# iammcy/BFLC-demo

Measured on AMD Instinct MI355X. Metric: fl_round_wall_clock_ms, lower is better.
Workload: dtype bf16; 1 GPU; model=femnist_cnn, global_batch=4096, img=1x28x28x62cls, parallelism=fl_nodes1, clients=8, update_quota=4, aggregate_top_k=3, samples_per_client=3072, batch_size=1024, partition=dirichlet, byzantine_clients=0

## Files before the change

### csrc/hip/bindings.cpp

```cpp
#include <torch/extension.h>

#include <string>
#include <tuple>
#include <vector>

namespace bflc {

void axpy_(torch::Tensor y, torch::Tensor x, double alpha);
void sgd_step_(torch::Tensor p, torch::Tensor g, double lr);
void adam_step_(torch::Tensor p, torch::Tensor g, torch::Tensor m,
                torch::Tensor v, long step, double lr, double beta1,
                double beta2, double eps);
torch::Tensor weighted_fedavg(torch::Tensor deltas, torch::Tensor w);
void sgd_master_(torch::Tensor p, torch::Tensor shadow, torch::Tensor g,
                 double lr);
void adam_master_(torch::Tensor p, torch::Tensor shadow, torch::Tensor g,
                  torch::Tensor m, torch::Tensor v, long step, double lr,
                  double beta1, double beta2, double eps);
void adam_master_graph_(torch::Tensor p, torch::Tensor shadow,
                        torch::Tensor g, torch::Tensor m, torch::Tensor v,
                        torch::Tensor step, torch::Tensor bc, double lr,
                        double beta1, double beta2, double eps);
void refresh_shadow_(torch::Tensor p, torch::Tensor shadow);
void score_load_(torch::Tensor shadow, torch::Tensor global_flat,
// ... 54 lines not shown
std::string conv_fwd_pool_impl(std::vector<long> x_shape,
                               std::vector<long> w_shape, long stride,
                               long pad);
long halo_conv_group_images_query(std::vector<long> x_shape,
                                  std::vector<long> w_shape, long stride,
                                  long pad);
std::string conv2d_relu_pool_route(std::vector<long> x_shape,
                                   std::vector<long> w_shape, long stride,
                                   long pad);
PlanRow conv_plan_route(const std::string& entry, std::vector<long> x_shape,
                        std::vector<long> w_shape, long stride, long pad);
std::tuple<torch::Tensor, torch::Tensor> conv2d_relu_pool_fwd_idx(
    torch::Tensor x, torch::Tensor w, torch::Tensor b, long stride,
    long pad, long max_blocks, std::string impl);
std::tuple<torch::Tensor, torch::Tensor> pool_relu_bwd_colsum(
    torch::Tensor y_pooled, torch::Tensor idx, torch::Tensor dy_pooled,
    std::vector<long> out_shape);
std::tuple<torch::Tensor, torch::Tensor> thin_conv_pool_wgrad(
    torch::Tensor x, torch::Tensor y_pooled, torch::Tensor idx,
    torch::Tensor dy_pooled, long stride, long pad);
std::tuple<torch::Tensor, torch::Tensor> thin_conv_pool_wgrad_fused(
    torch::Tensor x, torch::Tensor y_pooled, torch::Tensor idx,
    torch::Tensor dy_pooled, long stride, long pad);
std::string thin_pool_wgrad_impl(std::vector<long> x_shape,
                                 std::vector<long> w_shape, long stride,
                                 long pad, bool want_dx);
std::string conv2d_relu_pool_bwd_route(std::vector<long> x_shape,
                                       std::vector<long> w_shape,
                                       long stride, long pad, bool want_dx,
                                       bool allow_direct);
std::tuple<torch::Tensor, torch::Tensor, torch::Tensor> conv2d_relu_pool_bwd(
    torch::Tensor x, torch::Tensor w, torch::Tensor y_pooled,
    torch::Tensor idx, torch::Tensor dy_pooled, long stride, long pad,
    bool want_db, bool want_dx, bool allow_direct);

std::tuple<torch::Tensor, torch::Tensor, torch::Tensor> batchnorm_fwd(
    torch::Tensor x, torch::Tensor gamma, torch::Tensor beta, double eps,
    bool relu, c10::optional<torch::Tensor> residual);
std::tuple<torch::Tensor, torch::Tensor, torch::Tensor> batchnorm_bwd(
    torch::Tensor x, torch::Tensor dy, torch::Tensor mean,
    torch::Tensor invstd, torch::Tensor gamma,
    c10::optional<torch::Tensor> y_relu);
torch::Tensor global_avgpool_fwd(torch::Tensor x);
torch::Tensor global_avgpool_bwd(torch::Tensor dy, long H, long W);
torch::Tensor add_relu_fwd(torch::Tensor a, torch::Tensor b);
torch::Tensor add_relu_bwd(torch::Tensor y, torch::Tensor dy);

std::tuple<torch::Tensor, torch::Tensor, torch::Tensor> groupnorm_fwd(
    torch::Tensor x, torch::Tensor gamma, torch::Tensor beta, long groups,
    double eps, bool relu, c10::optional<torch::Tensor> residual);
std::tuple<torch::Tensor, torch::Tensor, torch::Tensor> groupnorm_bwd(
    torch::Tensor x, torch::Tensor dy, torch::Tensor mean, torch::Tensor rstd,
    torch::Tensor gamma, long groups, c10::optional<torch::Tensor> y_relu);
std::string groupnorm_route(long H, long W, long C, long groups);

}

PYBIND11_MODULE(TORCH_EXTENSION_NAME, m) {
  m.doc() = "bflc_amd hand-written gfx950 (CDNA4) HIP kernels";
  m.def("axpy_", &bflc::axpy_, "y += alpha*x (fp32, in place)");
  m.def("sgd_step_", &bflc::sgd_step_, "fused flat SGD");
  m.def("adam_step_", &bflc::adam_step_, "fused flat Adam");
  m.def("weighted_fedavg", &bflc::weighted_fedavg,
        "fixed-order weighted FedAvg reduce");
  m.def("sgd_master_", &bflc::sgd_master_,
        "fused fp32-master SGD + bf16 shadow refresh");
  m.def("adam_master_", &bflc::adam_master_);
// ... 83 lines not shown
        "route conv2d_relu_pool_fwd takes: gemm256_pool | thin_pool | "
        "unfused",
        py::arg("x_shape"), py::arg("w_shape"), py::arg("stride"),
        py::arg("pad"));
  m.def("conv2d_relu_pool_fwd_idx", &bflc::conv2d_relu_pool_fwd_idx,
        "training conv + bias + ReLU + 2x2/2 maxpool: (y_pooled, idx), "
        "same routes and options as conv2d_relu_pool_fwd",
        py::arg("x"), py::arg("w"), py::arg("b"), py::arg("stride"),
        py::arg("pad"), py::arg("max_blocks") = 0, py::arg("impl") = "");
  m.def("pool_relu_bwd_colsum", &bflc::pool_relu_bwd_colsum,
        "unpool + ReLU mask + bias grad in one pass: (dy_full_masked, db)",
        py::arg("y_pooled"), py::arg("idx"), py::arg("dy_pooled"),
        py::arg("out_shape"));
  m.def("thin_conv_pool_wgrad", &bflc::thin_conv_pool_wgrad,
        "direct first-layer (dw, db) from the pooled tensors",
        py::arg("x"), py::arg("y_pooled"), py::arg("idx"),
        py::arg("dy_pooled"), py::arg("stride"), py::arg("pad"));
  m.def("thin_conv_pool_wgrad_fused", &bflc::thin_conv_pool_wgrad_fused,
        "first-layer (dw, db) from the pooled tensors, bitwise the "
        "materialised unpool -> im2col -> split-K GEMM chain",
        py::arg("x"), py::arg("y_pooled"), py::arg("idx"),
        py::arg("dy_pooled"), py::arg("stride"), py::arg("pad"));
  m.def("thin_pool_wgrad_impl", &bflc::thin_pool_wgrad_impl,
        "what the unpool route runs for the thin first layer: "
        "fused_mfma | materialized",
        py::arg("x_shape"), py::arg("w_shape"), py::arg("stride"),
        py::arg("pad"), py::arg("want_dx"));
  m.def("conv2d_relu_pool_bwd_route", &bflc::conv2d_relu_pool_bwd_route,
        "route conv2d_relu_pool_bwd takes: thin_direct | unpool",
        py::arg("x_shape"), py::arg("w_shape"), py::arg("stride"),
        py::arg("pad"), py::arg("want_dx"), py::arg("allow_direct") = true);
  m.def("conv2d_relu_pool_bwd", &bflc::conv2d_relu_pool_bwd,
        "(dx, dw, db) of the fused conv + ReLU + pool from its saved "
        "(x, w, y_pooled, idx)",
        py::arg("x"), py::arg("w"), py::arg("y_pooled"), py::arg("idx"),
        py::arg("dy_pooled"), py::arg("stride"), py::arg("pad"),
        py::arg("want_db") = true, py::arg("want_dx") = true,
        py::arg("allow_direct") = true);
  m.def("batchnorm_fwd", &bflc::batchnorm_fwd,
        py::arg("x"), py::arg("gamma"), py::arg("beta"), py::arg("eps"),
        py::arg("relu"), py::arg("residual") = py::none(),
        "(y, mean, invstd) — batch-stats BN, optional fused relu");
  m.def("batchnorm_bwd", &bflc::batchnorm_bwd, "(dx, dgamma, dbeta)",
        py::arg("x"), py::arg("dy"), py::arg("mean"), py::arg("invstd"),
        py::arg("gamma"), py::arg("y_relu") = py::none());
  m.def("global_avgpool_fwd", &bflc::global_avgpool_fwd);
  m.def("global_avgpool_bwd", &bflc::global_avgpool_bwd);
  m.def("add_relu_fwd", &bflc::add_relu_fwd, "fused residual add + relu");
  m.def("add_relu_bwd", &bflc::add_relu_bwd);
  m.def("groupnorm_fwd", &bflc::groupnorm_fwd,
        py::arg("x"), py::arg("gamma"), py::arg("beta"), py::arg("groups"),
        py::arg("eps"), py::arg("relu"), py::arg("residual") = py::none(),
        "(y, mean [N,G], rstd [N,G]) — per-sample GroupNorm, optional "
        "fused residual add + relu");
  m.def("groupnorm_bwd", &bflc::groupnorm_bwd, "(dx, dgamma, dbeta)",
        py::arg("x"), py::arg("dy"), py::arg("mean"), py::arg("rstd"),
        py::arg("gamma"), py::arg("groups"), py::arg("y_relu") = py::none());
  m.def("groupnorm_route", &bflc::groupnorm_route,
        "route groupnorm_fwd/bwd take: slab | split (from H, W, C, groups "
        "only — never N)",
        py::arg("H"), py::arg("W"), py::arg("C"), py::arg("groups"));
}
```

### csrc/hip/conv2d.hip

```cpp

#include "common.h"
#include "gemm_api.h"

namespace bflc {

namespace {

typedef __attribute__((ext_vector_type(8))) __bf16 bf16x8_t;
typedef __attribute__((ext_vector_type(8))) unsigned short u16x8_t;
typedef __attribute__((ext_vector_type(8))) int i32x8_t;
typedef __attribute__((ext_vector_type(4))) float f32x4_t;

__global__ void im2col_nhwc_vec_kernel(const bf16* __restrict__ x,
                                       bf16* __restrict__ col, ConvShape sh,
                                       long total_g) {
  const int c8g = sh.C / 8;
  const int rs = sh.R * sh.S;
  long g = (long)blockIdx.x * blockDim.x + threadIdx.x;
  const long stride = (long)gridDim.x * blockDim.x;
  for (; g < total_g; g += stride) {
    const int c8 = (int)(g % c8g) * 8;
    const int k = (int)((g / c8g) % rs);
    const long m = g / ((long)c8g * rs);
    const int s = k % sh.S, r = k / sh.S;
// ... 787 lines not shown

torch::Tensor conv2d_fwd(torch::Tensor x, torch::Tensor w, torch::Tensor b,
                         long stride, long pad, bool relu) {
  return std::get<0>(conv2d_fwd_col(x, w, b, stride, pad, relu, false));
}

std::tuple<torch::Tensor, torch::Tensor, torch::Tensor, torch::Tensor>
conv2d_fwd_bn(torch::Tensor x, torch::Tensor w, long stride, long pad) {
  CHECK_GPU(x); CHECK_CONTIG(x); CHECK_CONTIG(w);
  auto sh = make_shape(x, w, stride, pad);
  auto w2 = w.view({(long)sh.Kout, sh.RSC()});
  auto y = torch::empty({(long)sh.N, (long)sh.OH, (long)sh.OW,
                         (long)sh.Kout}, x.options());
  std::pair<torch::Tensor, torch::Tensor> stats;
  auto none = torch::empty({0}, x.options());
  if (is_1x1_s1(sh)) {
    auto col = x.view({sh.M(), (long)sh.C});
    gemm_bf16_raw(col, w2, y, sh.M(), sh.Kout, sh.RSC(), false, true,
                  nullptr, false, EpStore::kPlain, 0, &stats);
    return {y, col, stats.first.defined() ? stats.first : none,
            stats.second.defined() ? stats.second : none};
  }
  if (gemm_conv_fwd_raw(x, w2, y, sh, nullptr, false, &stats))
    return {y, none, stats.first.defined() ? stats.first : none,
            stats.second.defined() ? stats.second : none};
  auto col = im2col(x, sh);
  const long kp = col.size(1);
  gemm_bf16_raw(col, pad_w2(w2, kp), y, sh.M(), sh.Kout, kp, false, true,
                nullptr, false, EpStore::kPlain, 0, &stats);
  return {y, col, stats.first.defined() ? stats.first : none,
          stats.second.defined() ? stats.second : none};
}

std::tuple<torch::Tensor, torch::Tensor, torch::Tensor> conv2d_bwd(
    torch::Tensor x, torch::Tensor w, torch::Tensor dy, long stride,
    long pad, c10::optional<torch::Tensor> col_cache, bool want_db,
    bool want_dx) {
  CHECK_GPU(x); CHECK_CONTIG(x); CHECK_CONTIG(w); CHECK_CONTIG(dy);
  auto sh = make_shape(x, w, stride, pad);
  auto w2 = w.view({(long)sh.Kout, sh.RSC()});
  auto dy2 = dy.view({sh.M(), (long)sh.Kout});

  torch::Tensor dx;
  bool dgrad_done = !want_dx;
  if (!want_dx) {
    dx = torch::empty({0}, x.options());
  } else if (is_1x1_s1(sh)) {
    auto wT = transpose_bf16(w2);
    dx = torch::empty_like(x);
    auto dxv = dx.view({sh.M(), (long)sh.C});
    gemm_bf16_raw(dy2, wT, dxv, sh.M(), sh.RSC(), sh.Kout, false, true,
                  nullptr, false, EpStore::kPlain, 0);
    dgrad_done = true;
  } else if (sh.Kout % 8 == 0 && sh.C <= dgrad_implicit_max_c() &&
             sh.C >= 8 && sh.stride == 1) {
    auto wrot2 = w.permute({3, 1, 2, 0}).contiguous()
                     .view({(long)sh.C, (long)sh.R * sh.S * sh.Kout});
    dx = torch::empty_like(x);
    auto dxv = dx.view({(long)sh.N * sh.H * sh.W, (long)sh.C});
    dgrad_done = gemm_conv_dgrad_raw(dy2, wrot2, dxv, sh);
  }
  if (!dgrad_done) {
    auto wT = transpose_bf16(w2);
    auto dcol = torch::empty({sh.M(), sh.RSC()}, x.options());
    gemm_bf16_raw(dy2, wT, dcol, sh.M(), sh.RSC(), sh.Kout, false, true,
                  nullptr, false, EpStore::kPlain, 0);
    dx = torch::empty_like(x);
    if (sh.C % 8 == 0) {
      const long total_g = (long)sh.N * sh.H * sh.W * (sh.C / 8);
      hipLaunchKernelGGL(col2im_nhwc_vec_kernel, dim3(ew_grid(total_g)),
                         dim3(256), 0, cur_stream(),
                         (const bf16*)dcol.data_ptr(),
                         (bf16*)dx.data_ptr(), sh, total_g);
    } else {
      const long total = dx.numel();
      hipLaunchKernelGGL(col2im_nhwc_kernel, dim3(ew_grid(total)), dim3(256),
                         0, cur_stream(), (const bf16*)dcol.data_ptr(),
                         (bf16*)dx.data_ptr(), sh, total);
    }
    HIP_CHECK(hipGetLastError());
  }

  auto dw = torch::empty_like(w2);
  bool wgrad_done = false;
  if (!is_1x1_s1(sh) && sh.Kout <= wgrad_implicit_max_kout() &&
      !(col_cache.has_value() && col_cache->numel() > 0))
    wgrad_done = gemm_conv_wgrad_raw(dy2, x, dw, sh);
  if (!wgrad_done) {
    auto col = (col_cache.has_value() && col_cache->numel() > 0)
                   ? *col_cache
                   : (is_1x1_s1(sh) ? x.view({sh.M(), (long)sh.C})
                                    : im2col(x, sh));
    const long kp = col.size(1);
    if (kp == sh.RSC()) {
      gemm_bf16_raw(dy2, col, dw, sh.Kout, sh.RSC(), sh.M(), true, false,
                    nullptr, false, EpStore::kPlain, 0);
    } else {
      auto dwp = torch::empty({(long)sh.Kout, kp}, dw.options());
      gemm_bf16_raw(dy2, col, dwp, sh.Kout, kp, sh.M(), true, false,
                    nullptr, false, EpStore::kPlain, 0);
      dw.copy_(dwp.slice(1, 0, sh.RSC()));
    }
  }

  auto db = want_db ? colsum_bf16(dy2)
                    : torch::empty({0}, dy.options());
  return {dx, dw.view(w.sizes()), db};
}

std::tuple<torch::Tensor, torch::Tensor> maxpool2d_fwd(torch::Tensor x,
                                                       long kernel,
                                                       long stride,
                                                       bool want_idx) {
  CHECK_GPU(x); CHECK_CONTIG(x);
  ConvShape sh;
  sh.N = (int)x.size(0); sh.H = (int)x.size(1);
  sh.W = (int)x.size(2); sh.C = (int)x.size(3);
  sh.R = sh.S = (int)kernel; sh.stride = (int)stride; sh.pad = 0;
  sh.Kout = sh.C;
  sh.OH = (sh.H - sh.R) / sh.stride + 1;
  sh.OW = (sh.W - sh.S) / sh.stride + 1;
  auto y = torch::empty({(long)sh.N, (long)sh.OH, (long)sh.OW, (long)sh.C},
                        x.options());
  TORCH_CHECK(sh.R * sh.S <= 255, "maxpool window too large for u8 idx");
  const bool skip_idx = !want_idx && sh.C % 8 == 0;
  auto idx = skip_idx
                 ? torch::empty({0}, y.options().dtype(at::kByte))
                 : torch::empty_like(y, y.options().dtype(at::kByte));
  if (sh.C % 8 == 0) {
    const long total_g = sh.M() * (sh.C / 8);
    hipLaunchKernelGGL(maxpool_nhwc_vec_fwd, dim3(ew_grid(total_g)),
                       dim3(256), 0, cur_stream(),
                       (const bf16*)x.data_ptr(), (bf16*)y.data_ptr(),
                       skip_idx ? nullptr : idx.data_ptr<uint8_t>(), sh,
                       total_g);
  } else {
    const long total = y.numel();
    hipLaunchKernelGGL(maxpool_nhwc_fwd, dim3(ew_grid(total)), dim3(256), 0,
                       cur_stream(), (const bf16*)x.data_ptr(),
                       (bf16*)y.data_ptr(), idx.data_ptr<uint8_t>(), sh,
// ... 121 lines not shown
  bool ok = false;
  long S = 1, kslice = 0;
  int tbl_pairs = 0;
  long lds = 0;
  int cshift = 0;
};

ThinFusedPlan thin_fused_plan(const ConvShape& sh) {
  ThinFusedPlan t;
  if (!thin_wgrad_eligible(sh) || sh.N <= 0) return t;
  const long Mpix = sh.M();
  const long kp = (sh.RSC() + 7) / 8 * 8;
  const GemmPlan p = gemm_dense_plan(sh.Kout, kp, Mpix, true, false);
  const long lim = 1L << 31;
  if (p.path != GemmPath::kSmall || kp != 16 || Mpix * sh.Kout >= lim ||
      (long)sh.N * sh.H * sh.W >= lim || (long)sh.N * (sh.OH + 2) >= lim)
    return t;
  t.S = p.S;
  t.kslice = p.kslice;
  int rows_max = 0;
  for (long s = 0; s < p.S; ++s) {
    int P0, rows;
    thin_wgrad_window(sh, s * p.kslice,
                      std::min(Mpix, (s + 1) * p.kslice), &P0, &rows);
    rows_max = std::max(rows_max, rows);
  }
  const long xelems = (long)(rows_max + 2) * (sh.OW + 2) + 4;
  const long pairs = (p.kslice / 32 + 1) * 16;
  t.tbl_pairs = (int)pairs;
  t.lds = pairs * 8 + (xelems + 1) / 2 * 4;
  while (t.cshift < 6 && (1 << t.cshift) < sh.OW + 2) ++t.cshift;
  t.ok = t.lds <= kThinFusedMaxLds && xelems <= 32768;
  return t;
}

}

torch::Tensor conv2d_relu_pool_fwd(torch::Tensor x, torch::Tensor w,
                                   torch::Tensor b, long stride, long pad,
                                   long max_blocks, std::string impl) {
  return std::get<0>(
      relu_pool_fwd_impl(x, w, b, stride, pad, false, max_blocks, impl));
}

std::string conv_fwd_pool_impl(std::vector<long> x_shape,
                               std::vector<long> w_shape, long stride,
                               long pad) {
  const auto sh = make_shape_dims(x_shape, w_shape, stride, pad);
  return pool_route(sh) == PoolRoute::kGemm256 && halo_conv_gate(sh)
             ? "halo_mfma"
             : "gemm256";
}

long halo_conv_group_images_query(std::vector<long> x_shape,
                                  std::vector<long> w_shape, long stride,
                                  long pad) {
  return halo_conv_group_images(
      make_shape_dims(x_shape, w_shape, stride, pad));
}

std::tuple<torch::Tensor, torch::Tensor> conv2d_relu_pool_fwd_idx(
    torch::Tensor x, torch::Tensor w, torch::Tensor b, long stride,
    long pad, long max_blocks, std::string impl) {
  return relu_pool_fwd_impl(x, w, b, stride, pad, true, max_blocks, impl);
}

// ... 57 lines not shown
                     (const bf16*)y_pooled.data_ptr(),
                     idx.data_ptr<uint8_t>(),
                     (const bf16*)dy_pooled.data_ptr(), sh, MP, G, rows,
                     part.data_ptr<float>());
  HIP_CHECK(hipGetLastError());
  hipLaunchKernelGGL(thin_conv_pool_wgrad_final_kernel,
                     dim3(ceil_div((long)N * kWgradAcc, 4)), dim3(256), 0,
                     cur_stream(), part.data_ptr<float>(), chunks, N,
                     (bf16*)dw.data_ptr(), (bf16*)db.data_ptr());
  HIP_CHECK(hipGetLastError());
  return {dw, db};
}

std::tuple<torch::Tensor, torch::Tensor> thin_conv_pool_wgrad_fused(
    torch::Tensor x, torch::Tensor y_pooled, torch::Tensor idx,
    torch::Tensor dy_pooled, long stride, long pad) {
  CHECK_GPU(x); CHECK_CONTIG(x);
  TORCH_CHECK(x.scalar_type() == at::kBFloat16 && x.dim() == 4,
              "thin_conv_pool_wgrad_fused: bf16 NHWC x");
  check_pooled(y_pooled, idx, dy_pooled);
  const auto sh = make_shape_dims(
      x.sizes().vec(), {y_pooled.size(3), 3, 3, x.size(3)}, stride, pad);
  const ThinFusedPlan t = thin_fused_plan(sh);
  TORCH_CHECK(t.ok,
              "thin_conv_pool_wgrad_fused: 3x3, C == 1, stride 1, even "
              "OH/OW, Kout % 8 == 0 and Kout <= 64, on the small-tile "
              "split-K plan, only");
  TORCH_CHECK(y_pooled.size(0) == sh.N && y_pooled.size(1) == sh.OH / 2 &&
              y_pooled.size(2) == sh.OW / 2,
              "thin_conv_pool_wgrad_fused: pooled shape does not match x");
  const long Mpix = sh.M();
  const int N = sh.Kout;
  auto dw = torch::empty({(long)N, 3, 3, 1}, x.options());
  auto db = torch::empty({(long)N}, x.options());

  torch::Tensor part;
  if (t.S > 1)
    part = torch::empty({t.S, (long)N, 9}, x.options().dtype(at::kFloat));
  const int frags = (N + 15) / 16;
  auto* kern = frags <= 2 ? thin_pool_wgrad_mfma_kernel<4>
                          : thin_pool_wgrad_mfma_kernel<2>;
  hipLaunchKernelGGL(kern, dim3((unsigned)t.S),
                     dim3(frags * (frags <= 2 ? 4 : 2) * 64), (size_t)t.lds,
                     cur_stream(), (const unsigned short*)x.data_ptr(),
                     (const unsigned short*)y_pooled.data_ptr(),
                     idx.data_ptr<uint8_t>(),
                     (const unsigned short*)dy_pooled.data_ptr(), sh, Mpix,
                     t.kslice, t.cshift, t.tbl_pairs,
                     t.S > 1 ? part.data_ptr<float>() : nullptr,
                     (bf16*)dw.data_ptr());
  HIP_CHECK(hipGetLastError());
  if (t.S > 1) {
    auto dw2 = dw.view({(long)N, 9});
    splitk_reduce_plain(part, dw2);
  }

  const ColsumGeom g = colsum_geom(Mpix, N);
  auto cpart = torch::empty({g.chunks, (long)N},
                            x.options().dtype(at::kFloat));
  hipLaunchKernelGGL(pool_relu_bwd_colsum_part_kernel<false>,
                     dim3(g.cblocks, g.chunks), dim3(256), 0, cur_stream(),
                     (const bf16*)y_pooled.data_ptr(),
                     idx.data_ptr<uint8_t>(),
                     (const bf16*)dy_pooled.data_ptr(), (bf16*)nullptr, Mpix,
                     (long)N, sh.OH, sh.OW, g.G, g.rows,
                     cpart.data_ptr<float>());
  HIP_CHECK(hipGetLastError());
  colsum_finalize(cpart, db);
  return {dw, db};
}

std::string thin_pool_wgrad_impl(std::vector<long> x_shape,
                                 std::vector<long> w_shape, long stride,
                                 long pad, bool want_dx) {
  const auto sh = make_shape_dims(x_shape, w_shape, stride, pad);
  return !want_dx && thin_fused_wgrad_gate() && thin_fused_plan(sh).ok
             ? "fused_mfma"
             : "materialized";
}

std::string conv2d_relu_pool_bwd_route(std::vector<long> x_shape,
                                       std::vector<long> w_shape,
                                       long stride, long pad, bool want_dx,
                                       bool allow_direct) {
  const auto sh = make_shape_dims(x_shape, w_shape, stride, pad);
  return allow_direct && !want_dx && thin_wgrad_eligible(sh) ? "thin_direct"
                                                             : "unpool";
}

std::tuple<torch::Tensor, torch::Tensor, torch::Tensor> conv2d_relu_pool_bwd(
    torch::Tensor x, torch::Tensor w, torch::Tensor y_pooled,
    torch::Tensor idx, torch::Tensor dy_pooled, long stride, long pad,
    bool want_db, bool want_dx, bool allow_direct) {
  CHECK_GPU(x); CHECK_CONTIG(x); CHECK_CONTIG(w);
  const auto sh = make_shape(x, w, stride, pad);
  TORCH_CHECK(sh.OH % 2 == 0 && sh.OW % 2 == 0 &&
              y_pooled.dim() == 4 && y_pooled.size(0) == sh.N &&
              y_pooled.size(1) == sh.OH / 2 &&
              y_pooled.size(2) == sh.OW / 2 && y_pooled.size(3) == sh.Kout,
              "conv2d_relu_pool_bwd: pooled shape does not match the conv");
  auto none = torch::empty({0}, x.options());
  if (allow_direct && !want_dx && thin_wgrad_eligible(sh)) {
    auto [dw, db] = thin_conv_pool_wgrad(x, y_pooled, idx, dy_pooled,
                                         stride, pad);
    return {none, dw.view(w.sizes()), want_db ? db : none};
  }
  if (!want_dx && thin_fused_wgrad_gate() && thin_fused_plan(sh).ok) {
    auto [dw, db] = thin_conv_pool_wgrad_fused(x, y_pooled, idx, dy_pooled,
                                               stride, pad);
    return {none, dw.view(w.sizes()), want_db ? db : none};
  }
  auto [dyf, db] = pool_relu_bwd_colsum(
      y_pooled, idx, dy_pooled,
      {(long)sh.N, (long)sh.OH, (long)sh.OW, (long)sh.Kout});
  auto [dx, dw, db_unused] =
      conv2d_bwd(x, w, dyf, stride, pad, c10::nullopt, false, want_dx);
  (void)db_unused;
  return {dx, dw, want_db ? db : none};
}

torch::Tensor maxpool2d_bwd(torch::Tensor dy, torch::Tensor idx,
                            std::vector<long> in_shape, long kernel,
                            long stride) {
  CHECK_GPU(dy); CHECK_CONTIG(dy); CHECK_CONTIG(idx);
  TORCH_CHECK(idx.numel() == dy.numel(),
              "maxpool2d_bwd: argmax mask missing/size-mismatched (the "
              "forward ran with want_idx=false?)");
  ConvShape sh;
  sh.N = (int)in_shape[0]; sh.H = (int)in_shape[1];
  sh.W = (int)in_shape[2]; sh.C = (int)in_shape[3];
  sh.R = sh.S = (int)kernel; sh.stride = (int)stride; sh.pad = 0;
  sh.Kout = sh.C;
  sh.OH = (int)dy.size(1); sh.OW = (int)dy.size(2);
  auto dx = torch::empty({(long)sh.N, (long)sh.H, (long)sh.W, (long)sh.C},
                         dy.options());
  if (sh.C % 8 == 0) {
    const long total_g = (long)sh.N * sh.H * sh.W * (sh.C / 8);
    hipLaunchKernelGGL(maxpool_nhwc_vec_bwd, dim3(ew_grid(total_g)),
                       dim3(256), 0, cur_stream(),
                       (const bf16*)dy.data_ptr(), idx.data_ptr<uint8_t>(),
                       (bf16*)dx.data_ptr(), sh, total_g);
  } else {
    const long total = dx.numel();
// ... 11 lines not shown
```

### csrc/hip/gemm_api.h

```cpp
#pragma once

#include <torch/extension.h>

#include <string>
#include <tuple>

#include "gemm_plan.h"

namespace bflc {

#if defined(__HIPCC__) || defined(__HIP__)
#define BFLC_HD __host__ __device__
#else
#define BFLC_HD
#endif

struct ConvShape {
  int N, C, H, W, Kout, R, S, stride, pad, OH, OW;
  BFLC_HD long M() const { return (long)N * OH * OW; }
  BFLC_HD long RSC() const { return (long)R * S * C; }
};

enum class EpStore : int {
  kPlain = 0,
// ... 14 lines not shown
PlanRow gemm_plan_route(long M, long N, long K, bool ta, bool tb);
GemmPlan gemm_dense_plan(long M, long N, long K, bool ta, bool tb);
void splitk_reduce_plain(const torch::Tensor& part, torch::Tensor& out);

enum class ConvEntry { kFwd, kFwdPool, kDgrad, kWgrad };
GemmPlan gemm_conv_plan(ConvEntry e, const ConvShape& sh);

bool gemm_thin_conv_raw(const torch::Tensor& x, const torch::Tensor& w2p,
                        torch::Tensor& y, const ConvShape& sh,
                        const torch::Tensor* bias, bool relu);

bool gemm_conv_fwd_raw(const torch::Tensor& x, const torch::Tensor& w2,
                       torch::Tensor& y, const ConvShape& sh,
                       const torch::Tensor* bias, bool relu,
                       std::pair<torch::Tensor, torch::Tensor>* bn_stats
                       = nullptr);

bool gemm_conv_fwd_pool_eligible(const ConvShape& sh);
enum class HaloMode { kAuto, kOff, kForce };
bool gemm_conv_fwd_pool_raw(const torch::Tensor& x, const torch::Tensor& w2,
                            torch::Tensor& y, const ConvShape& sh,
                            const torch::Tensor* bias, bool relu,
                            uint8_t* idx = nullptr,
                            HaloMode halo = HaloMode::kAuto,
                            int max_blocks = 0);

bool halo_conv_geometry_ok(const ConvShape& sh);
int halo_conv_group_images(const ConvShape& sh);
bool halo_conv_gate(const ConvShape& sh);
void halo_conv_fwd_pool_launch(const torch::Tensor& x,
                               const torch::Tensor& w2, torch::Tensor& y,
                               const ConvShape& sh, const torch::Tensor* bias,
                               bool relu, uint8_t* idx, int max_blocks);
bool gemm_thin_conv_pool_eligible(const ConvShape& sh, long KT);
bool gemm_thin_conv_pool_raw(const torch::Tensor& x,
                             const torch::Tensor& w2p, torch::Tensor& y,
                             const ConvShape& sh, const torch::Tensor* bias,
                             bool relu, uint8_t* idx = nullptr);

bool gemm_conv_dgrad_raw(const torch::Tensor& dy, const torch::Tensor& wrot2,
                         torch::Tensor& dx, const ConvShape& sh);

bool gemm_conv_wgrad_raw(const torch::Tensor& dy2, const torch::Tensor& x,
                         torch::Tensor& dw, const ConvShape& sh);

torch::Tensor colsum_bf16(const torch::Tensor& X);
void colsum_finalize(const torch::Tensor& part, torch::Tensor& out);
std::tuple<torch::Tensor, torch::Tensor> relu_bwd_colsum(
    const torch::Tensor& y, const torch::Tensor& dy);

torch::Tensor transpose_bf16(const torch::Tensor& X);

}
```

### csrc/hip/halo_conv.hip

```cpp
#include "common.h"
#include "gemm_api.h"

#include <cstdlib>

namespace bflc {

namespace {

typedef __attribute__((ext_vector_type(8))) __bf16 bf16x8_t;
typedef __attribute__((ext_vector_type(4))) unsigned int u32x4_t;
typedef __attribute__((ext_vector_type(4))) float f32x4_t;

constexpr int kHaloThreads = 256;
constexpr int kHaloWC = 1;
constexpr int kHaloPF = 8;
constexpr int kHaloMinBlocks = 2;
constexpr long kHaloLdsBudget = 80 * 1024;

struct Magic { unsigned long long m; };
inline Magic make_magic(unsigned d) { return {0xFFFFFFFFull / d + 1}; }
__device__ __forceinline__ unsigned mdiv(unsigned n, Magic g) {
  return (unsigned)(((unsigned long long)n * g.m) >> 32);
}

// ... 169 lines not shown

bool halo_conv_env_gate() {
  static const bool v = [] {
    const char* e = getenv("BFLC_HALO_CONV");
    return (e ? atoi(e) : 1) != 0;
  }();
  return v;
}

struct HaloGeom {
  bool ok = false;
  int G = 0, pitch = 0, img_lds = 0;
};

HaloGeom halo_geom(const ConvShape& sh) {
  HaloGeom g;
  if (sh.C != 32 || sh.R != 3 || sh.S != 3 || sh.stride != 1 ||
      sh.pad != 1 || sh.Kout != 64 || sh.N <= 0 || sh.OH <= 0 ||
      sh.OW <= 0 || sh.OH % 2 != 0 || sh.OW % 2 != 0)
    return g;
  g.pitch = (sh.W + 2) * 64 + 32;
  const long img = (long)(sh.H + 2) * g.pitch;
  const long by_lds = kHaloLdsBudget / (2 * img);
  const long by_pf =
      (long)kHaloPF * kHaloThreads / ((long)sh.H * sh.W * 4);
  const long G = std::min(by_lds, by_pf);
  if (G < 1) return g;
  g.G = (int)G;
  g.img_lds = (int)img;
  g.ok = true;
  return g;
}

}

bool halo_conv_geometry_ok(const ConvShape& sh) { return halo_geom(sh).ok; }

int halo_conv_group_images(const ConvShape& sh) { return halo_geom(sh).G; }

bool halo_conv_gate(const ConvShape& sh) {
  if (!halo_conv_env_gate() || !halo_geom(sh).ok) return false;
  const GemmPlan p = gemm_conv_plan(ConvEntry::kFwdPool, sh);
  return p.path == GemmPath::kGemm256 && p.S == 1;
}

void halo_conv_fwd_pool_launch(const torch::Tensor& x,
                               const torch::Tensor& w2, torch::Tensor& y,
                               const ConvShape& sh, const torch::Tensor* bias,
                               bool relu, uint8_t* idx, int max_blocks) {
  const HaloGeom g = halo_geom(sh);
  TORCH_CHECK(g.ok, "halo conv: shape outside the kernel's geometry");
  TORCH_CHECK((long)sh.N * sh.H * sh.W * 64 < (1L << 40), "halo conv: N");
  HaloParams p;
  p.N = sh.N; p.H = sh.H; p.W = sh.W;
  p.PH = sh.OH / 2; p.PW = sh.OW / 2;
  p.G = g.G; p.pitch = g.pitch; p.img_lds = g.img_lds;
  p.hw4 = sh.H * sh.W * 4;
  p.phw = p.PH * p.PW;
  p.m_hw4 = make_magic((unsigned)p.hw4);
  p.m_w = make_magic((unsigned)p.W);
  p.m_phw = make_magic((unsigned)p.phw);
  p.m_pw = make_magic((unsigned)p.PW);
  const size_t lds = (size_t)2 * g.G * g.img_lds;
  const int groups = (sh.N + g.G - 1) / g.G;
  int blocks = std::min(groups, kHaloMinBlocks * kNumCU);
  if (max_blocks > 0) blocks = std::min(blocks, max_blocks);
// ... 21 lines not shown
```

Baseline: 5.434 ms/round.

## Add fused halo MFMA dgrad kernel for conv+relu+pool backward

Result: faster. 5.092 ms/round (median of 6 runs) (-6.3%).

```diff
diff --git a/csrc/hip/bindings.cpp b/csrc/hip/bindings.cpp
--- a/csrc/hip/bindings.cpp
+++ b/csrc/hip/bindings.cpp
@@ -110,7 +110,17 @@
 std::tuple<torch::Tensor, torch::Tensor, torch::Tensor> conv2d_relu_pool_bwd(
     torch::Tensor x, torch::Tensor w, torch::Tensor y_pooled,
     torch::Tensor idx, torch::Tensor dy_pooled, long stride, long pad,
-    bool want_db, bool want_dx, bool allow_direct);
+    bool want_db, bool want_dx, bool allow_direct, std::string dgrad_impl,
+    long max_blocks);
+std::string pool_dgrad_impl(std::vector<long> x_shape,
+                            std::vector<long> w_shape, long stride, long pad,
+                            bool want_dx);
+long halo_dgrad_group_images_query(std::vector<long> x_shape,
+                                   std::vector<long> w_shape, long stride,
+                                   long pad);
+std::tuple<torch::Tensor, torch::Tensor> halo_pool_dgrad(
+    torch::Tensor w, torch::Tensor y_pooled, torch::Tensor idx,
+    torch::Tensor dy_pooled, long max_blocks, bool store_plane);
 
 std::tuple<torch::Tensor, torch::Tensor, torch::Tensor> batchnorm_fwd(
     torch::Tensor x, torch::Tensor gamma, torch::Tensor beta, double eps,
@@ -260,11 +270,30 @@
         py::arg("pad"), py::arg("want_dx"), py::arg("allow_direct") = true);
   m.def("conv2d_relu_pool_bwd", &bflc::conv2d_relu_pool_bwd,
         "(dx, dw, db) of the fused conv + ReLU + pool from its saved "
-        "(x, w, y_pooled, idx)",
+        "(x, w, y_pooled, idx). dgrad_impl pins halo_mfma | implicit_gemm "
+        "('' = pool_dgrad_impl's answer); max_blocks > 0 caps the halo "
+        "kernel's grid",
         py::arg("x"), py::arg("w"), py::arg("y_pooled"), py::arg("idx"),
         py::arg("dy_pooled"), py::arg("stride"), py::arg("pad"),
         py::arg("want_db") = true, py::arg("want_dx") = true,
-        py::arg("allow_direct") = true);
+        py::arg("allow_direct") = true, py::arg("dgrad_impl") = "",
+        py::arg("max_blocks") = 0);
+  m.def("pool_dgrad_impl", &bflc::pool_dgrad_impl,
+        "data gradient the unpool route runs: halo_mfma | implicit_gemm",
+        py::arg("x_shape"), py::arg("w_shape"), py::arg("stride"),
+        py::arg("pad"), py::arg("want_dx"));
+  m.def("halo_dgrad_group_images", &bflc::halo_dgrad_group_images_query,
+        "images per LDS group of the halo dgrad kernel (0: not its "
+        "geometry)",
+        py::arg("x_shape"), py::arg("w_shape"), py::arg("stride"),
+        py::arg("pad"));
+  m.def("halo_pool_dgrad", &bflc::halo_pool_dgrad,
+        "the halo dgrad kernel on its geometry alone: (dx, masked "
+        "full-resolution dy plane) from w and the pooled (y, idx, dy); "
+        "store_plane = false skips the plane store (0-size plane)",
+        py::arg("w"), py::arg("y_pooled"), py::arg("idx"),
+        py::arg("dy_pooled"), py::arg("max_blocks") = 0,
+        py::arg("store_plane") = true);
   m.def("batchnorm_fwd", &bflc::batchnorm_fwd,
         py::arg("x"), py::arg("gamma"), py::arg("beta"), py::arg("eps"),
         py::arg("relu"), py::arg("residual") = py::none(),
diff --git a/csrc/hip/conv2d.hip b/csrc/hip/conv2d.hip
--- a/csrc/hip/conv2d.hip
+++ b/csrc/hip/conv2d.hip
@@ -843,15 +843,12 @@
           stats.second.defined() ? stats.second : none};
 }
 
-std::tuple<torch::Tensor, torch::Tensor, torch::Tensor> conv2d_bwd(
-    torch::Tensor x, torch::Tensor w, torch::Tensor dy, long stride,
-    long pad, c10::optional<torch::Tensor> col_cache, bool want_db,
-    bool want_dx) {
-  CHECK_GPU(x); CHECK_CONTIG(x); CHECK_CONTIG(w); CHECK_CONTIG(dy);
-  auto sh = make_shape(x, w, stride, pad);
+namespace {
+
+torch::Tensor conv_dgrad(const torch::Tensor& x, const torch::Tensor& w,
+                         const torch::Tensor& dy2, const ConvShape& sh,
+                         bool want_dx) {
   auto w2 = w.view({(long)sh.Kout, sh.RSC()});
-  auto dy2 = dy.view({sh.M(), (long)sh.Kout});
-
   torch::Tensor dx;
   bool dgrad_done = !want_dx;
   if (!want_dx) {
@@ -891,7 +888,13 @@
     }
     HIP_CHECK(hipGetLastError());
   }
-
+  return dx;
+}
+
+torch::Tensor conv_wgrad(const torch::Tensor& x, const torch::Tensor& w,
+                         const torch::Tensor& dy2, const ConvShape& sh,
+                         const c10::optional<torch::Tensor>& col_cache) {
+  auto w2 = w.view({(long)sh.Kout, sh.RSC()});
   auto dw = torch::empty_like(w2);
   bool wgrad_done = false;
   if (!is_1x1_s1(sh) && sh.Kout <= wgrad_implicit_max_kout() &&
@@ -913,10 +916,24 @@
       dw.copy_(dwp.slice(1, 0, sh.RSC()));
     }
   }
+  return dw.view(w.sizes());
+}
+
+}
+
+std::tuple<torch::Tensor, torch::Tensor, torch::Tensor> conv2d_bwd(
+    torch::Tensor x, torch::Tensor w, torch::Tensor dy, long stride,
+    long pad, c10::optional<torch::Tensor> col_cache, bool want_db,
+    bool want_dx) {
+  CHECK_GPU(x); CHECK_CONTIG(x); CHECK_CONTIG(w); CHECK_CONTIG(dy);
+  auto sh = make_shape(x, w, stride, pad);
+  auto dy2 = dy.view({sh.M(), (long)sh.Kout});
+  auto dx = conv_dgrad(x, w, dy2, sh, want_dx);
+  auto dw = conv_wgrad(x, w, dy2, sh, col_cache);
 
   auto db = want_db ? colsum_bf16(dy2)
                     : torch::empty({0}, dy.options());
-  return {dx, dw.view(w.sizes()), db};
+  return {dx, dw, db};
 }
 
 std::tuple<torch::Tensor, torch::Tensor> maxpool2d_fwd(torch::Tensor x,
@@ -1104,6 +1121,28 @@
   while (t.cshift < 6 && (1 << t.cshift) < sh.OW + 2) ++t.cshift;
   t.ok = t.lds <= kThinFusedMaxLds && xelems <= 32768;
   return t;
+}
+
+torch::Tensor pool_relu_bwd_db(const torch::Tensor& y_pooled,
+                               const torch::Tensor& idx,
+                               const torch::Tensor& dy_pooled,
+                               const ConvShape& sh) {
+  const long Mpix = sh.M();
+  const long N = sh.Kout;
+  TORCH_CHECK(Mpix * N < (1L << 31), "pool_relu_bwd_db: 32-bit indices");
+  auto db = torch::empty({N}, dy_pooled.options());
+  const ColsumGeom g = colsum_geom(Mpix, N);
+  auto cpart = torch::empty({g.chunks, N},
+                            dy_pooled.options().dtype(at::kFloat));
+  hipLaunchKernelGGL(pool_relu_bwd_colsum_part_kernel<false>,
+                     dim3(g.cblocks, g.chunks), dim3(256), 0, cur_stream(),
+                     (const bf16*)y_pooled.data_ptr(),
+                     idx.data_ptr<uint8_t>(),
+                     (const bf16*)dy_pooled.data_ptr(), (bf16*)nullptr, Mpix,
+                     N, sh.OH, sh.OW, g.G, g.rows, cpart.data_ptr<float>());
+  HIP_CHECK(hipGetLastError());
+  colsum_finalize(cpart, db);
+  return db;
 }
 
 }
@@ -1227,7 +1266,7 @@
   const long Mpix = sh.M();
   const int N = sh.Kout;
   auto dw = torch::empty({(long)N, 3, 3, 1}, x.options());
-  auto db = torch::empty({(long)N}, x.options());
+  torch::Tensor db;
 
   torch::Tensor part;
   if (t.S > 1)
@@ -1250,18 +1289,7 @@
     splitk_reduce_plain(part, dw2);
   }
 
-  const ColsumGeom g = colsum_geom(Mpix, N);
-  auto cpart = torch::empty({g.chunks, (long)N},
-                            x.options().dtype(at::kFloat));
-  hipLaunchKernelGGL(pool_relu_bwd_colsum_part_kernel<false>,
-                     dim3(g.cblocks, g.chunks), dim3(256), 0, cur_stream(),
-                     (const bf16*)y_pooled.data_ptr(),
-                     idx.data_ptr<uint8_t>(),
-                     (const bf16*)dy_pooled.data_ptr(), (bf16*)nullptr, Mpix,
-                     (long)N, sh.OH, sh.OW, g.G, g.rows,
-                     cpart.data_ptr<float>());
-  HIP_CHECK(hipGetLastError());
-  colsum_finalize(cpart, db);
+  db = pool_relu_bwd_db(y_pooled, idx, dy_pooled, sh);
   return {dw, db};
 }
 
@@ -1283,10 +1311,63 @@
                                                              : "unpool";
 }
 
+namespace {
+
+std::tuple<torch::Tensor, torch::Tensor> halo_pool_dgrad_impl(
+    const torch::Tensor& x_like, const torch::Tensor& w,
+    const torch::Tensor& y_pooled, const torch::Tensor& idx,
+    const torch::Tensor& dy_pooled, const ConvShape& sh, long max_blocks,
+    bool store_plane = true) {
+  auto dyf = store_plane
+                 ? torch::empty({(long)sh.N, (long)sh.OH, (long)sh.OW,
+                                 (long)sh.Kout}, dy_pooled.options())
+                 : torch::empty({0}, dy_pooled.options());
+  auto dx = torch::empty({(long)sh.N, (long)sh.H, (long)sh.W, (long)sh.C},
+                         x_like.options());
+  halo_pool_dgrad_launch(w, y_pooled, idx, dy_pooled,
+                         store_plane ? &dyf : nullptr, dx, sh,
+                         (int)max_blocks);
+  return {dx, dyf};
+}
+
+}
+
+std::string pool_dgrad_impl(std::vector<long> x_shape,
+                            std::vector<long> w_shape, long stride, long pad,
+                            bool want_dx) {
+  const auto sh = make_shape_dims(x_shape, w_shape, stride, pad);
+  return want_dx && halo_dgrad_gate(sh) ? "halo_mfma" : "implicit_gemm";
+}
+
+long halo_dgrad_group_images_query(std::vector<long> x_shape,
+                                   std::vector<long> w_shape, long stride,
+                                   long pad) {
+  return halo_dgrad_group_images(
+      make_shape_dims(x_shape, w_shape, stride, pad));
+}
+
+std::tuple<torch::Tensor, torch::Tensor> halo_pool_dgrad(
+    torch::Tensor w, torch::Tensor y_pooled, torch::Tensor idx,
+    torch::Tensor dy_pooled, long max_blocks, bool store_plane) {
+  CHECK_GPU(w); CHECK_CONTIG(w);
+  TORCH_CHECK(w.scalar_type() == at::kBFloat16 && w.dim() == 4,
+              "halo_pool_dgrad: bf16 KRSC w");
+  check_pooled(y_pooled, idx, dy_pooled);
+  const auto sh = make_shape_dims(
+      {y_pooled.size(0), 2 * y_pooled.size(1), 2 * y_pooled.size(2),
+       w.size(3)},
+      w.sizes().vec(), 1, 1);
+  TORCH_CHECK(y_pooled.size(3) == sh.Kout && halo_dgrad_geometry_ok(sh),
+              "halo_pool_dgrad: shape outside the halo kernel's geometry");
+  return halo_pool_dgrad_impl(dy_pooled, w, y_pooled, idx, dy_pooled, sh,
+                              max_blocks, store_plane);
+}
+
 std::tuple<torch::Tensor, torch::Tensor, torch::Tensor> conv2d_relu_pool_bwd(
     torch::Tensor x, torch::Tensor w, torch::Tensor y_pooled,
     torch::Tensor idx, torch::Tensor dy_pooled, long stride, long pad,
-    bool want_db, bool want_dx, bool allow_direct) {
+    bool want_db, bool want_dx, bool allow_direct, std::string dgrad_impl,
+    long max_blocks) {
   CHECK_GPU(x); CHECK_CONTIG(x); CHECK_CONTIG(w);
   const auto sh = make_shape(x, w, stride, pad);
   TORCH_CHECK(sh.OH % 2 == 0 && sh.OW % 2 == 0 &&
@@ -1294,6 +1375,15 @@
               y_pooled.size(1) == sh.OH / 2 &&
               y_pooled.size(2) == sh.OW / 2 && y_pooled.size(3) == sh.Kout,
               "conv2d_relu_pool_bwd: pooled shape does not match the conv");
+  TORCH_CHECK(dgrad_impl.empty() || dgrad_impl == "halo_mfma" ||
+                  dgrad_impl == "implicit_gemm",
+              "conv2d_relu_pool_bwd: dgrad_impl is '' | halo_mfma | "
+              "implicit_gemm");
+  const bool force_halo = dgrad_impl == "halo_mfma";
+  TORCH_CHECK(!force_halo || (want_dx && halo_dgrad_geometry_ok(sh) &&
+                              sh.M() * sh.Kout < (1L << 31)),
+              "conv2d_relu_pool_bwd: shape outside the halo dgrad kernel's "
+              "geometry");
   auto none = torch::empty({0}, x.options());
   if (allow_direct && !want_dx && thin_wgrad_eligible(sh)) {
     auto [dw, db] = thin_conv_pool_wgrad(x, y_pooled, idx, dy_pooled,
@@ -1304,6 +1394,16 @@
     auto [dw, db] = thin_conv_pool_wgrad_fused(x, y_pooled, idx, dy_pooled,
                                                stride, pad);
     return {none, dw.view(w.sizes()), want_db ? db : none};
+  }
+  if (force_halo ||
+      (dgrad_impl.empty() && want_dx && halo_dgrad_gate(sh))) {
+    check_pooled(y_pooled, idx, dy_pooled);
+    auto db = want_db ? pool_relu_bwd_db(y_pooled, idx, dy_pooled, sh) : none;
+    auto [dx, dyf] = halo_pool_dgrad_impl(x, w, y_pooled, idx, dy_pooled, sh,
+                                          max_blocks);
+    auto dy2 = dyf.view({sh.M(), (long)sh.Kout});
+    auto dw = conv_wgrad(x, w, dy2, sh, c10::nullopt);
+    return {dx, dw, db};
   }
   auto [dyf, db] = pool_relu_bwd_colsum(
       y_pooled, idx, dy_pooled,
diff --git a/csrc/hip/gemm_api.h b/csrc/hip/gemm_api.h
--- a/csrc/hip/gemm_api.h
+++ b/csrc/hip/gemm_api.h
@@ -70,6 +70,15 @@
                                const torch::Tensor& w2, torch::Tensor& y,
                                const ConvShape& sh, const torch::Tensor* bias,
                                bool relu, uint8_t* idx, int max_blocks);
+bool halo_dgrad_geometry_ok(const ConvShape& sh);
+int halo_dgrad_group_images(const ConvShape& sh);
+bool halo_dgrad_gate(const ConvShape& sh);
+void halo_pool_dgrad_launch(const torch::Tensor& w,
+                            const torch::Tensor& y_pooled,
+                            const torch::Tensor& idx,
+                            const torch::Tensor& dy_pooled,
+                            torch::Tensor* dyf, torch::Tensor& dx,
+                            const ConvShape& sh, int max_blocks);
 bool gemm_thin_conv_pool_eligible(const ConvShape& sh, long KT);
 bool gemm_thin_conv_pool_raw(const torch::Tensor& x,
                              const torch::Tensor& w2p, torch::Tensor& y,
diff --git a/csrc/hip/halo_conv.hip b/csrc/hip/halo_conv.hip
--- a/csrc/hip/halo_conv.hip
+++ b/csrc/hip/halo_conv.hip
@@ -225,6 +225,300 @@
   return g;
 }
 
+constexpr int kDgPF = 2;
+constexpr int kDgWPitch = 72;
+constexpr long kDgWBytes = 9L * 32 * kDgWPitch * 2;
+
+struct DgradParams {
+  int N, H, W, PW;
+  int G;
+  int WP;
+  int img_pix;
+  int hw;
+  int pgr;
+  Magic m_pgr8, m_pw, m_hw, m_w;
+};
+
+typedef __attribute__((ext_vector_type(8))) unsigned short u16x8_t;
+typedef __attribute__((ext_vector_type(2))) unsigned int u32x2_t;
+
+__device__ __forceinline__ int dg_lds_off(int pix, int slot) {
+  return pix * 128 + ((slot ^ ((pix >> 1) & 7)) << 4);
+}
+
+template <bool PLANE>
+__launch_bounds__(kHaloThreads, kHaloMinBlocks * (kHaloThreads / 256))
+__global__ void halo_pool_dgrad_kernel(const bf16* __restrict__ w,
+                                       const unsigned char* __restrict__ yp,
+                                       const unsigned char* __restrict__ idx,
+                                       const unsigned char* __restrict__ dyp,
+                                       unsigned char* __restrict__ dyf,
+                                       bf16* __restrict__ dx, DgradParams p) {
+  extern __shared__ __align__(16) unsigned char smem[];
+  constexpr int WR = kHaloThreads / 64;
+  constexpr int FN = 2, C = 32;
+
+  const int tid = threadIdx.x;
+  const int lane = tid & 63;
+  const int l15 = lane & 15, l4 = lane >> 4;
+  const int wave = __builtin_amdgcn_readfirstlane(tid >> 6);
+
+  const int buf_bytes = p.G * p.img_pix * 128;
+  const int ngroups = (p.N + p.G - 1) / p.G;
+  int g = blockIdx.x;
+  if (g >= ngroups) return;
+
+  int st_pix[kDgPF], st_gl[kDgPF];
+#pragma unroll
+  for (int i = 0; i < kDgPF; ++i) {
+    const unsigned gi = tid + i * kHaloThreads;
+    const unsigned pp = gi >> 3;
+    const unsigned img = mdiv(pp, p.m_pgr8);
+    const unsigned rem = pp - img * (p.pgr >> 3);
+    const unsigned ph = mdiv(rem, p.m_pw), pw = rem - ph * p.PW;
+    st_pix[i] = (int)(img * p.img_pix + (2 * ph + 1) * p.WP + 2 * pw + 1);
+    st_gl[i] = (int)((img * p.hw + 2 * ph * p.W + 2 * pw) * 8 + (gi & 7));
+  }
+  u32x4_t pf_dy[kDgPF], pf_y[kDgPF];
+  u32x2_t pf_ix[kDgPF];
+  auto fetch = [&](int gg) __attribute__((always_inline)) {
+    const int gc = min(p.G, p.N - gg * p.G);
+    const int ngr = gc * p.pgr;
+    const long base = (long)gg * p.G * p.pgr;
+#pragma unroll
+    for (int i = 0; i < kDgPF; ++i) {
+      const int gi = tid + i * kHaloThreads;
+      if (gi < ngr) {
+        pf_dy[i] =
+            *reinterpret_cast<const u32x4_t*>(dyp + (base + gi) * 16);
+        pf_y[i] = *reinterpret_cast<const u32x4_t*>(yp + (base + gi) * 16);
+        pf_ix[i] = *reinterpret_cast<const u32x2_t*>(idx + (base + gi) * 8);
+      }
+    }
+    return ngr;
+  };
+  auto stage = [&](int buf, int gg, int ngr) __attribute__((always_inline)) {
+    unsigned char* lbuf = smem + buf * buf_bytes;
+    unsigned char* gbase = dyf + (long)gg * p.G * p.hw * 128;
+    const bf16 zero = f2b(0.f);
+#pragma unroll
+    for (int i = 0; i < kDgPF; ++i) {
+      const int gi = tid + i * kHaloThreads;
+      if (gi < ngr) {
+        const bf16x8_t dv = __builtin_bit_cast(bf16x8_t, pf_dy[i]);
+        const bf16x8_t yv = __builtin_bit_cast(bf16x8_t, pf_y[i]);
+        const unsigned long long iv =
+            __builtin_bit_cast(unsigned long long, pf_ix[i]);
+        const int slot = gi & 7;
+#pragma unroll
+        for (int q = 0; q < 4; ++q) {
+          bf16x8_t gv;
+#pragma unroll
+          for (int j = 0; j < 8; ++j) {
+            float a = 0.f;
+            if ((int)((iv >> (8 * j)) & 0xff) == q) a += b2f(dv[j]);
+            gv[j] = f2b(a);
+            if (!(b2f(yv[j]) > 0.f)) gv[j] = zero;
+          }
+          const int pix = st_pix[i] + (q >> 1) * p.WP + (q & 1);
+          *reinterpret_cast<bf16x8_t*>(lbuf + dg_lds_off(pix, slot)) = gv;
+          if (PLANE) {
+            const long go = st_gl[i] + ((q >> 1) * p.W + (q & 1)) * 8;
+            *reinterpret_cast<bf16x8_t*>(gbase + go * 16) = gv;
+          }
+        }
+      }
+    }
+  };
+
+  int ngr0 = fetch(g);
+
+  {
+    unsigned short* wt = reinterpret_cast<unsigned short*>(smem);
+    const unsigned short* wg = reinterpret_cast<const unsigned short*>(w);
+    const int kout = lane;
+    u16x8_t wv[9];
+#pragma unroll
+    for (int i = 0; i < 9; ++i) {
+      const int q = wave + i * WR;
+      wv[i] = *reinterpret_cast<const u16x8_t*>(&wg[kout * 288 + q * 8]);
+    }
+#pragma unroll
+    for (int i = 0; i < 9; ++i) {
+      const int q = wave + i * WR;
+#pragma unroll
+      for (int j = 0; j < 8; ++j) wt[(q * 8 + j) * kDgWPitch + kout] = wv[i][j];
+    }
+  }
+  __syncthreads();
+  bf16x8_t bfr[9][2][FN];
+  {
+    const unsigned short* wt = reinterpret_cast<const unsigned short*>(smem);
+#pragma unroll
+    for (int t = 0; t < 9; ++t)
+#pragma unroll
+      for (int h = 0; h < 2; ++h)
+#pragma unroll
+        for (int fn = 0; fn < FN; ++fn)
+          bfr[t][h][fn] = *reinterpret_cast<const bf16x8_t*>(
+              &wt[(t * 32 + fn * 16 + l15) * kDgWPitch + h * 32 + l4 * 8]);
+  }
+  __syncthreads();
+
+  {
+    const u32x4_t z = {0u, 0u, 0u, 0u};
+    for (int o = tid * 16; o < 2 * buf_bytes; o += kHaloThreads * 16)
+      *reinterpret_cast<u32x4_t*>(smem + o) = z;
+  }
+  __syncthreads();
+  stage(0, g, ngr0);
+  __syncthreads();
+
+  int cur = 0;
+  for (; g < ngroups; g += gridDim.x) {
+    const int gnext = g + gridDim.x;
+    const bool has_next = gnext < ngroups;
+    int ngr_next = 0;
+    if (has_next) ngr_next = fetch(gnext);
+
+    const int gc = min(p.G, p.N - g * p.G);
+    const int npix = gc * p.hw;
+    const int ntiles = (npix + 15) >> 4;
+    const long m0 = (long)g * p.G * p.hw;
+    const unsigned char* lbuf = smem + cur * buf_bytes;
+
+    for (int mt = wave; mt < ntiles; mt += WR) {
+      const int m = mt * 16 + l15;
+      const unsigned mc = m < npix ? m : 0;
+      const unsigned img = mdiv(mc, p.m_hw);
+      const unsigned rem = mc - img * p.hw;
+      const unsigned ih = mdiv(rem, p.m_w), iw = rem - ih * p.W;
+      const int pix0 =
+          (int)(img * p.img_pix + (ih + 2) * p.WP + iw + 2);
+
+      f32x4_t acc[FN] = {};
+#pragma unroll
+      for (int t = 0; t < 9; ++t) {
+        const int r = t / 3, s = t - r * 3;
+        const int off = dg_lds_off(pix0 - r * p.WP - s, l4);
+#pragma unroll
+        for (int h = 0; h < 2; ++h) {
+          const bf16x8_t af =
+              *reinterpret_cast<const bf16x8_t*>(lbuf + (off ^ (h << 6)));
+#pragma unroll
+          for (int fn = 0; fn < FN; ++fn)
+            acc[fn] = __builtin_amdgcn_mfma_f32_16x16x32_bf16(
+                af, bfr[t][h][fn], acc[fn], 0, 0, 0);
+        }
+      }
+
+#pragma unroll
+      for (int r = 0; r < 4; ++r) {
+        const int row = mt * 16 + l4 * 4 + r;
+        if (row < npix) {
+#pragma unroll
+          for (int fn = 0; fn < FN; ++fn)
+            dx[(m0 + row) * C + fn * 16 + l15] = f2b(acc[fn][r] + 0.f);
+        }
+      }
+    }
+
+    if (has_next) stage(cur ^ 1, gnext, ngr_next);
+    __syncthreads();
+    cur ^= 1;
+  }
+}
+
+bool halo_dgrad_env_gate() {
+  static const bool v = [] {
+    const char* e = getenv("BFLC_HALO_DGRAD");
+    return (e ? atoi(e) : 1) != 0;
+  }();
+  return v;
+}
+
+struct DgradGeom {
+  bool ok = false;
+  int G = 0;
+  long img_lds = 0;
+};
+
+DgradGeom dgrad_geom(const ConvShape& sh) {
+  DgradGeom g;
+  if (sh.C != 32 || sh.R != 3 || sh.S != 3 || sh.stride != 1 ||
+      sh.pad != 1 || sh.Kout != 64 || sh.N <= 0 || sh.OH <= 0 ||
+      sh.OW <= 0 || sh.OH % 2 != 0 || sh.OW % 2 != 0)
+    return g;
+  g.img_lds = (long)(sh.OH + 2) * (sh.OW + 2) * 128;
+  const long by_lds = kHaloLdsBudget / (2 * g.img_lds);
+  const long by_pf =
+      (long)kDgPF * kHaloThreads / ((long)(sh.OH / 2) * (sh.OW / 2) * 8);
+  const long G = std::min(by_lds, by_pf);
+  if (G < 1) return g;
+  g.G = (int)G;
+  g.ok = true;
+  return g;
+}
+
+}
+
+bool halo_dgrad_geometry_ok(const ConvShape& sh) { return dgrad_geom(sh).ok; }
+
+int halo_dgrad_group_images(const ConvShape& sh) { return dgrad_geom(sh).G; }
+
+bool halo_dgrad_gate(const ConvShape& sh) {
+  if (!halo_dgrad_env_gate() || !dgrad_geom(sh).ok) return false;
+  if (sh.M() * sh.Kout >= (1L << 31)) return false;
+  const GemmPlan p = gemm_conv_plan(ConvEntry::kDgrad, sh);
+  return p.path != GemmPath::kNone && p.S == 1;
+}
+
+void halo_pool_dgrad_launch(const torch::Tensor& w,
+                            const torch::Tensor& y_pooled,
+                            const torch::Tensor& idx,
+                            const torch::Tensor& dy_pooled,
+                            torch::Tensor* dyf, torch::Tensor& dx,
+                            const ConvShape& sh, int max_blocks) {
+  const DgradGeom g = dgrad_geom(sh);
+  TORCH_CHECK(g.ok, "halo dgrad: shape outside the kernel's geometry");
+  TORCH_CHECK((long)sh.N * sh.OH * sh.OW < (1L << 31), "halo dgrad: N");
+  DgradParams p;
+  p.N = sh.N; p.H = sh.OH; p.W = sh.OW; p.PW = sh.OW / 2;
+  p.G = g.G;
+  p.WP = sh.OW + 2;
+  p.img_pix = (sh.OH + 2) * (sh.OW + 2);
+  p.hw = sh.OH * sh.OW;
+  p.pgr = (sh.OH / 2) * (sh.OW / 2) * 8;
+  p.m_pgr8 = make_magic((unsigned)(p.pgr / 8));
+  p.m_pw = make_magic((unsigned)p.PW);
+  p.m_hw = make_magic((unsigned)p.hw);
+  p.m_w = make_magic((unsigned)p.W);
+  const size_t lds =
+      (size_t)std::max<long>(2L * g.G * g.img_lds, kDgWBytes);
+  const int groups = (sh.N + g.G - 1) / g.G;
+  int blocks = std::min(groups, kHaloMinBlocks * kNumCU);
+  if (max_blocks > 0) blocks = std::min(blocks, max_blocks);
+  static const bool attr_set = [] {
+    HIP_CHECK(hipFuncSetAttribute(
+        (const void*)halo_pool_dgrad_kernel<true>,
+        hipFuncAttributeMaxDynamicSharedMemorySize, (int)kHaloLdsBudget));
+    HIP_CHECK(hipFuncSetAttribute(
+        (const void*)halo_pool_dgrad_kernel<false>,
+        hipFuncAttributeMaxDynamicSharedMemorySize, (int)kHaloLdsBudget));
+    return true;
+  }();
+  (void)attr_set;
+  auto* kern = dyf ? halo_pool_dgrad_kernel<true>
+                   : halo_pool_dgrad_kernel<false>;
+  hipLaunchKernelGGL(kern, dim3((unsigned)blocks),
+                     dim3(kHaloThreads), lds, cur_stream(),
+                     (const bf16*)w.data_ptr(),
+                     (const unsigned char*)y_pooled.data_ptr(),
+                     (const unsigned char*)idx.data_ptr(),
+                     (const unsigned char*)dy_pooled.data_ptr(),
+                     dyf ? (unsigned char*)dyf->data_ptr() : nullptr,
+                     (bf16*)dx.data_ptr(), p);
+  HIP_CHECK(hipGetLastError());
 }
 
 bool halo_conv_geometry_ok(const ConvShape& sh) { return halo_geom(sh).ok; }
```
